# AER-RC/RRTMG_LW

Measured on AMD Instinct MI355X. Metric: columns/sec, 72-layer profiles, higher is better.
Workload: dtype f64 (transmittance / tfn codes and their LDS table f32); 1 GPU; 1000000 synthetic 72-layer columns, config 'cloudy' (icld=2: rtrnmr max-random overlap, idrv=0), sharded 1x1000000; ncol_total=1000000, nlay=72, columns_per_gpu=1000000, parallelism=columns/1, gather=none, kdata=stand-in (real k-data absent from the reference mount), sweeps=production

## Files before the change

### rrtmg_lw_amd/csrc/driver.hip

```cpp
#include <hip/hip_runtime.h>
#include <cstdlib>
#include <sched.h>

#include <algorithm>
#include <array>
#include <atomic>
#include <cstdint>
#include <cstdarg>
#include <mutex>
#include <string>
#include <chrono>
#include <condition_variable>
#include <functional>
#include <map>
#include <thread>
#include <type_traits>
#include <vector>

#include "../../include/rrtmg_lw_hip.h"
#include "kernels.hip"
#include "mtjump.hpp"
#include "hostrows.hpp"
#include "owned.hpp"

// ... 2 lines not shown
using namespace rrlw;

constexpr int BLOCK = 256;
const int HOST_BATCH = []() { const char *e = getenv("RRTMG_LW_HOST_BATCH"); const int v = e ? atoi(e) : 0; return v >= 64 ? v : 16384; }();

constexpr int HOST_SETS = 4;

struct DevMemTraits {
    using handle = void *;
    static int acquire(void **p, size_t bytes) { return (int)hipMalloc(p, bytes); }
    static int release(void *p) { const hipError_t s = hipDeviceSynchronize(), f = hipFree(p); return (int)(s != hipSuccess ? s : f); }
};
struct PinnedTraits {
    using handle = void *;
    static int acquire(void **p, size_t bytes) { return (int)hipHostMalloc(p, bytes, hipHostMallocDefault); }
    static int release(void *p) { return (int)hipHostFree(p); }
};
struct StreamTraits { using handle = hipStream_t; static int release(hipStream_t s) { return (int)hipStreamDestroy(s); } };
struct EventTraits { using handle = hipEvent_t; static int release(hipEvent_t e) { return (int)hipEventDestroy(e); } };
struct GraphTraits { using handle = hipGraph_t; static int release(hipGraph_t g) { return (int)hipGraphDestroy(g); } };
struct GraphExecTraits { using handle = hipGraphExec_t; static int release(hipGraphExec_t g) { return (int)hipGraphExecDestroy(g); } };
using DevBuf = owned::GrowBuf<DevMemTraits>;
using PinnedBuf = owned::GrowBuf<PinnedTraits>;
using Stream = owned::Owned<StreamTraits>;
using Event = owned::Owned<EventTraits>;
using Graph = owned::Owned<GraphTraits>;
using GraphExec = owned::Owned<GraphExecTraits>;

constexpr int KISS_SLOTS = 2 * RRTMG_LW_HIP_MAX_SAMPLES;
struct KissSlot { unsigned long long stride = 0; long long seed = -1; unsigned long long used = 0; };
struct KissTable { std::vector<KissSlot> slot; unsigned long long clock = 0; DevBuf dev; PinnedBuf host; };

constexpr int DEFAULT_BATCH = 262144;
struct State {
    bool init = false;
    int device = -1;
    HostTables H;
    DevTables D;
    DevBuf d_ktab, d_stat;
    Workspace W{};
    DevBuf ws_buf;
    struct WsShape {
        int nlay = 0, ncolb = 0;
        bool cloud = false, mc = false, gdp = false, efcl = false, ovl = false;
        bool two_scr = false;
        int groups = 0;
        size_t slabcols = 0;
    } ws;
    DevBuf opt_buf;
    int opt_nlay = 0, opt_ncolb = 0;
    double *opt_percol = nullptr;
    int *opt_laytrop = nullptr, *opt_wide = nullptr;
    DevBuf d_err;
    struct PrepSet { double *percol; int *laytrop, *ncbands; double *odcld, *efcl; int *cflag; int *btop, *order, *hgrp, *hblk, *bbot, *hbot; double2 *ovl; int *perm, *wsort; double *tlayc, *tlevc, *cldfc; int *wide; } prep[2] = {};
    struct ScrSet { unsigned *scr[NSCR]; unsigned *fw; } scrset[2] = {};
    Stream aux;
    struct SweepSet { Stream main, q[3]; Event go, done[3]; } swset[2];
    Stream lay_u, lay_m;
    int cu_layer = 0;
    int cu_total = 0;
    bool sweep_fanout = true;
    Event ev_last;
    Event ev_fork, ev_join;
    bool ev_last_valid = false;
    Event ev_in, ev_ready[2], ev_layer[2], ev_done[2];
    DevBuf mask;
    DevBuf d_rnd;
    bool batch_set = false;
    int batch = DEFAULT_BATCH;
    bool split_sweep = false;
    bool sweep_attrs = false;
    bool n1 = false;
    DevBuf stage_buf;
    DevBuf form_buf, form_gen;
    Stream stream;
    Stream cp_in, cp_out;
    PinnedBuf h_tot;
    struct HostSet { PinnedBuf in, out, fill, widen, narrow; } hset[HOST_SETS];
    Event ev_h2d[HOST_SETS], ev_cmp[HOST_SETS], ev_d2h[HOST_SETS];
    KissTable kiss;
    std::string err;
    bool profile = false;
    struct GraphEnt { std::vector<unsigned char> key; GraphExec exec; int seen = 0; bool failed = false; unsigned long long used = 0; };
    std::vector<GraphEnt> graphs;
    unsigned long long graph_clock = 0;
    Stream cap;
    long long graph_replays = 0, graph_captures = 0;
    unsigned long long init_gen = 0;
    struct ProfRec { const char *name; Event a, b; };
    std::vector<ProfRec> prof;
    std::vector<Event> evpool;
};
constexpr int MAXDEV = 16;
owned::NoDestroy<std::array<State, MAXDEV>> g_states_store;
std::array<State, MAXDEV> &g_states = g_states_store.get();
int g_ndev = 1;
thread_local State *g_cur = &g_states[0];
#define G (*g_cur)
std::mutex g_mu;

struct CallDesc {
    int ncol, nlay;
    int *icld;
    int idrv, inflg, iceflg, liqflg;
    int permuteseed = 0; int *irng = nullptr;
    bool spectral = false;
    size_t esz = 8;
// ... 345 lines not shown

void graphs_clear();
int g_split_max = []() { const char *e = getenv("RRTMG_LW_SPLIT_MAX"); return e ? std::max(0, atoi(e)) : 768; }();
int ensure_workspace(int nlay, int ncolb, bool cloud, bool mc = false, int idrv = 1, int mode = -1)
{
    SweepGroups fgw;
    int groups = NGROUP_MAX;
    if (mode >= 0 && make_groups(mode, idrv, 1, NBND, fgw)) groups = fgw.n;
    const bool gdp = idrv == 1, efcl = cloud && (mode < 0 || mode == 1 || mode == 3), ovl = cloud && (mode < 0 || mode == 2);
    const size_t split_cols = ncolb <= g_split_max ? (size_t)NBND * align_up((size_t)ncolb, 64) : 0;
    const State::WsShape &have = G.ws;
    if (G.ws_buf && have.nlay == nlay && have.ncolb >= ncolb && (have.cloud || !cloud) && (have.mc || !mc) && (have.two_scr || !G.split_sweep) &&
        have.groups >= groups && have.slabcols >= split_cols && (have.gdp || !gdp) && (have.efcl || !efcl) && (have.ovl || !ovl)) return 0;
    if (G.ws_buf) { HIP_TRY(hipDeviceSynchronize()); graphs_clear(); if (int rc = drop(G.ws_buf, "workspace")) return rc; }
    const bool same = have.nlay == nlay;
    ncolb = std::max(ncolb, same ? have.ncolb : 0);
    cloud = cloud || have.cloud || mc;
    mc = mc || have.mc;
    const int ng = std::max(groups, have.groups);
    const bool want_gdp = gdp || have.gdp, want_efcl = efcl || have.efcl, want_ovl = ovl || have.ovl;
    const size_t n = (size_t)ncolb, L = (size_t)nlay;
    const size_t slabcols = std::max((size_t)ng * n, (size_t)NBND * align_up(std::min(n, (size_t)std::max(g_split_max, 0)), 64));
    struct Item { void **p; size_t bytes; };
    Workspace &W = G.W;
    W = Workspace{};
    std::vector<Item> items = {
        {(void **)&W.gdn1, slabcols * (L + 1) * sizeof(double)},
        {(void **)&W.gup1, slabcols * (L + 1) * sizeof(double)},
        {(void **)&W.gup, slabcols * (L + 1) * sizeof(Part2)},
        {(void **)&W.gdn, slabcols * (L + 1) * sizeof(Part2)},
    };
    if (want_gdp) items.push_back({(void **)&W.gdp, slabcols * (L + 1) * sizeof(Part2)});
    const bool two_scr = G.split_sweep;
    G.scrset[1] = State::ScrSet{};
    for (int k = 0; k < (two_scr ? 2 : 1); k++) {
        State::ScrSet &ss = G.scrset[k];
        ss = State::ScrSet{};
        items.push_back({(void **)&ss.scr[S_CODE], (size_t)NQUAD * L * n * CODE_BYTES});
        items.push_back({(void **)&ss.fw, (size_t)NFW * L * n * sizeof(unsigned)});
        if (cloud) items.push_back({(void **)&ss.scr[S_CODET], (size_t)NQUAD * L * n * CODE_BYTES});
    }
    for (auto &ps : G.prep) {
        ps = State::PrepSet{};
        items.push_back({(void **)&ps.percol, (size_t)NPERCOL * n * 8});
        items.push_back({(void **)&ps.laytrop, n * 4});
        items.push_back({(void **)&ps.ncbands, n * 4});
        items.push_back({(void **)&ps.cflag, (L + 2) * n * 4});
        const size_t nblk = (n + 63) / 64, nslot = (size_t)sort_slots((int)nblk);
        items.push_back({(void **)&ps.btop, nblk * 4});
        items.push_back({(void **)&ps.hblk, nblk * 4});
        items.push_back({(void **)&ps.order, nslot * 4});
        items.push_back({(void **)&ps.hgrp, (nslot / SORT_GROUP) * 4});
        items.push_back({(void **)&ps.bbot, nblk * 4});
        items.push_back({(void **)&ps.hbot, (nslot / SORT_GROUP) * 4});
        items.push_back({(void **)&ps.perm, align_up(n, COLSORT_WIN) * 4});
        items.push_back({(void **)&ps.wsort, (align_up(n, COLSORT_WIN) / COLSORT_WIN) * 4});
        items.push_back({(void **)&ps.wide, (2 + ((n + LAYER_BLOCK - 1) / LAYER_BLOCK) * L) * 4});
        if (cloud) {
            items.push_back({(void **)&ps.tlayc, L * n * 8});
            items.push_back({(void **)&ps.tlevc, (L + 1) * n * 8});
            items.push_back({(void **)&ps.cldfc, L * n * 8});
        }
    }
    if (cloud) items.push_back({(void **)&W.hand, (size_t)5 * NQUAD * 4 * n * 8});
    if (cloud) {
        for (auto &ps : G.prep) {
            items.push_back({(void **)&ps.odcld, 16 * L * n * 8});
            if (want_efcl) items.push_back({(void **)&ps.efcl, 16 * L * n * 8});
            if (want_ovl) items.push_back({(void **)&ps.ovl, (size_t)2 * (L + 1) * 3 * n * sizeof(double2)});
        }
    }
    if (mc) {
        items.push_back({(void **)&W.odg, (size_t)NQUAD * 4 * L * n * 8});
        items.push_back({(void **)&W.cfef, (size_t)NQUAD * 8 * L * n * 4});
    }
    size_t total = 0;
    for (auto &it : items) total += align_up(it.bytes, 256);
    if (int rc = grow(G.ws_buf, total, total, "workspace")) return rc;
    size_t off = 0;
    for (auto &it : items) { *it.p = G.ws_buf.as<char>() + off; off += align_up(it.bytes, 256); }
    for (auto &ps : G.prep) HIP_TRY(hipMemset(ps.wide, 0, 8));
    W.ncolb = ncolb;
    W.pcb = ncolb;
    W.nlay = nlay;
    W.err = G.d_err.as<int>();
    for (int a = 0; a < NSCR; a++) W.scr[a] = G.scrset[0].scr[a];
    W.fw = G.scrset[0].fw;
    {
        const State::PrepSet &ps = G.prep[0];
        W.percol = ps.percol; W.laytrop = ps.laytrop; W.ncbands = ps.ncbands; W.cflag = ps.cflag;
        W.odcld = ps.odcld; W.efcl = ps.efcl; W.ovl = ps.ovl;
        W.btop = ps.btop; W.order = ps.order; W.hgrp = ps.hgrp; W.hblk = ps.hblk; W.bbot = ps.bbot; W.hbot = ps.hbot;
    }
    G.ws = State::WsShape{nlay, ncolb, cloud, mc, want_gdp, want_efcl, want_ovl, two_scr, ng, slabcols};
    return 0;
}

int ensure_mask(int nlay, size_t ncol)
{
    const size_t bytes = (size_t)KJ_NWORD * nlay * ncol * sizeof(unsigned);
    return grow(G.mask, bytes, bytes, "sub-column masks");
}

bool g_colsort = []() { const char *e = getenv("RRTMG_LW_COLSORT"); return !e || atoi(e) != 0; }();
bool use_colsort(bool gcm, int mode, int nb);
constexpr int COLSORT_NEVER = 1 << 24;
int g_colsort_min = []() { const char *e = getenv("RRTMG_LW_COLSORT_MIN"); return e ? std::max(0, std::min(atoi(e), COLSORT_NEVER)) : 24; }();
constexpr int COLSORT_CLEAR_MAX = 1000;
constexpr int COLSORT_CLEAR_DEFAULT = 18;
int g_colsort_clear = []() { const char *e = getenv("RRTMG_LW_COLSORT_CLEAR"); return e ? std::max(0, std::min(atoi(e), COLSORT_CLEAR_MAX)) : COLSORT_CLEAR_DEFAULT; }();
bool g_clear_groups = []() { const char *e = getenv("RRTMG_LW_CLEAR_GROUPS"); return !e || atoi(e) != 0; }();

Workspace ws_for(int k, bool sorted)
{
    Workspace w = G.W;
    const State::PrepSet &ps = G.prep[k];
    w.perm = sorted ? ps.perm : nullptr;
    w.wsort = sorted ? ps.wsort : nullptr;
    w.tlayc = ps.tlayc; w.tlevc = ps.tlevc; w.cldfc = ps.cldfc;
    w.wide = ps.wide;
    w.percol = ps.percol; w.laytrop = ps.laytrop; w.ncbands = ps.ncbands; w.cflag = ps.cflag;
    w.odcld = ps.odcld; w.efcl = ps.efcl; w.ovl = ps.ovl;
    w.btop = ps.btop; w.order = ps.order; w.hgrp = ps.hgrp; w.hblk = ps.hblk; w.bbot = ps.bbot; w.hbot = ps.hbot;
    const State::ScrSet &ss = G.scrset[G.ws.two_scr ? k : 0];
    for (int a = 0; a < NSCR; a++) w.scr[a] = ss.scr[a];
    w.fw = ss.fw;
    return w;
}

int make_stream(Stream &st, int lo, int hi)
{
    if (hi <= lo) { HIP_TRY(hipStreamCreateWithFlags(st.slot(), hipStreamNonBlocking)); return 0; }
    uint32_t mask[32] = {};
    const int nw = (G.cu_total + 31) / 32;
    for (int b = lo; b < hi && b < 1024; b++) mask[b >> 5] |= 1u << (b & 31);
    HIP_TRY(hipExtStreamCreateWithCUMask(st.slot(), (uint32_t)nw, mask));
    return 0;
}
int ensure_sweep_set(int k)
{
    if (G.swset[k].q[0]) return 0;
    const int lo = k == 1 ? G.cu_layer : 0, hi = k == 1 ? G.cu_total : 0;
    State::SweepSet SS;
    if (int rc = make_stream(SS.main, lo, hi)) return rc;
    for (int j = 0; j < 3; j++) {
        if (int rc = make_stream(SS.q[j], lo, hi)) return rc;
        if (int rc = make_event(SS.done[j])) return rc;
    }
    if (int rc = make_event(SS.go)) return rc;
    G.swset[k] = std::move(SS);
    return 0;
}

int g_one_sweep_max = []() { const char *e = getenv("RRTMG_LW_ONE_SWEEP_MAX"); return e ? atoi(e) : 4096; }();
bool one_sweep(int nb, int mode) { return mode != 0 && nb <= g_one_sweep_max; }
bool g_wide_window = []() { const char *e = getenv("RRTMG_LW_WIDE_WINDOW"); return !e || atoi(e) != 0; }();
bool g_prep_fork = []() { const char *e = getenv("RRTMG_LW_PREP_FORK"); return !e || atoi(e) != 0; }();
bool g_layer_split = []() { const char *e = getenv("RRTMG_LW_LAYER_SPLIT"); return !e || atoi(e) != 0; }();
bool use_colsort(bool gcm, int mode, int nb) { return g_colsort && gcm && (mode == 1 || mode == 2 || mode == 3) && !one_sweep(nb, mode); }

template <bool GCM>
int run_prep(hipStream_t s, const Workspace &Wk, const Batch &b, const GcmIn &g, const ColIn &c, hipStream_t side = nullptr)
{
    const dim3 cgrid1((b.nb + 63) / 64), cblock1(64);
    if (Wk.perm) {
        const dim3 wgrid((b.nb + COLSORT_WIN - 1) / COLSORT_WIN);
        LAUNCH("k_colsort", (k_colsort<GCM>), wgrid, dim3(COLSORT_WIN, COLSORT_TY), s, Wk, g, c, b.nb, b.col0, b.nct, g_colsort_min, (int)((long long)Wk.nlay * g_colsort_clear / 100));
    }
    const bool scan = b.mode == 1 || b.mode == 2, fork = scan && side && side != s;
    if (fork) {
        HIP_TRY(hipEventRecord(G.ev_fork.get(), s));
        HIP_TRY(hipStreamWaitEvent(side, G.ev_fork.get(), 0));
    }
    LAUNCH("k_colprep", (k_colprep<GCM>), cgrid1, cblock1, fork ? side : s, G.D, Wk, g, c, b.nb, b.col0, b.nct, b.idrv, b.istart, scan ? 0 : 1);
    if (fork) HIP_TRY(hipEventRecord(G.ev_join.get(), side));
    if (scan) {
// ... 3809 lines not shown
```

### rrtmg_lw_amd/csrc/kernels.hip

```cpp
#include <hip/hip_runtime.h>
#include "kissjump.hpp"

#ifdef RRLW_TUNE
#define RRLW_BF_TUNE 1u
#else
#define RRLW_BF_TUNE 0u
#endif
#ifdef RRLW_G256
#define RRLW_BF_G256 8u
#else
#define RRLW_BF_G256 0u
#endif
#if defined(RRLW_LAYER_BLOCK) || defined(RRLW_STAGE_DOUBLES) || defined(RRLW_LAYER_WAVES) || defined(RRLW_LOAD_CHUNK) || defined(RRLW_MINOR_WIN) || \
    defined(RRLW_COLSORT_WIN) || defined(RRLW_SWEEPC_P0) || defined(RRLW_SWEEPC_P2D) || defined(RRLW_SWEEPC_WAVES_CAP) || defined(RRLW_SWEEPC_CODES) || \
    defined(RRLW_SWEEPZ_WAVES_G1) || defined(RRLW_SWEEPZ_WAVES_IDRV) || defined(RRLW_LAYER_STAMPS) || \
    defined(RRLW_DBG_DUMP)
#define RRLW_BF_GEOMETRY 16u
#else
#define RRLW_BF_GEOMETRY 0u
#endif

#include <algorithm>
#include <type_traits>
#include <utility>

#include "tables.hpp"

namespace rrlw {

constexpr unsigned BUILD_FLAGS = RRLW_BF_TUNE | RRLW_BF_G256 | RRLW_BF_GEOMETRY;

struct DevTables {
    const double *ktab;
    const double *stat;
    BandLayout band[NBND];
    StaticLayout sl;
    double absice0[2], abscld1, absliq0;
    double delwave[NBND];
    double refrat[NBND][6];
    double heatfac, fluxfac, oneminus, bpade;
};

enum Field {
    F_FAC00, F_FAC01, F_FAC10, F_FAC11,
    F_COLH2O, F_COLCO2, F_COLO3, F_COLN2O, F_COLCO, F_COLCH4, F_COLO2, F_COLBRD,
    F_COLDRY, F_SELFFAC, F_SELFFRAC, F_FORFAC, F_FORFRAC, F_MINORFRAC, F_SCALEMINOR, F_SCALEMINORN2,
    F_PAVEL, F_WX1, F_WX2, F_WX3, F_WX4,
    NFIELD
};
enum PerCol { PC_PLANKBND = 0, PC_DPLANKBND = 16, PC_SECDIFF = 32, NPERCOL = 48 };
enum Scr { S_CODE, S_CODET, NSCR };
struct alignas(16) Part2 { double a, b; };

typedef float scr_t;
constexpr int CODE_WORDS = 4;
constexpr int CODE_BYTES = 4 * CODE_WORDS;

struct Workspace {
    int ncolb;
    int nlay;
    double *percol;
    int *laytrop;
    int *ncbands;
    double *odcld;
    double *efcl;
    int *cflag;
    double2 *ovl;
    int *btop;
    int *order;
    int *hgrp;
    int *hblk;
    int *bbot;
    int *hbot;
    double *hand;
    unsigned *scr[NSCR];
    unsigned *fw;
    double *gdn1, *gup1;
    Part2 *gup, *gdp, *gdn;
    int pcb;
    int *err;
    double *odg;
    float *cfef;
    unsigned *mask;
    size_t mask_stride;
    size_t mask_col0;
    int *wide;
    int *perm;
    int *wsort;
    double *tlayc, *tlevc, *cldfc;
};
#ifndef RRLW_COLSORT_WIN
#define RRLW_COLSORT_WIN 256
#endif
constexpr int COLSORT_WIN = RRLW_COLSORT_WIN;
__device__ __forceinline__ bool pmoved(const Workspace &W, int slot) { return W.perm && W.wsort[__builtin_amdgcn_readfirstlane(slot) / COLSORT_WIN] != 0; }
__device__ __forceinline__ int pcol(const Workspace &W, int slot)
{
    if (!W.perm) return slot;
    const int moved = W.wsort[__builtin_amdgcn_readfirstlane(slot) / COLSORT_WIN];
    return moved ? W.perm[slot] : slot;
}
__device__ __forceinline__ double col_load(const double *row, unsigned off8)
{
    typedef unsigned int u32x2c __attribute__((ext_vector_type(2)));
    const u32x2c v = __builtin_amdgcn_raw_buffer_load_b64(__builtin_amdgcn_make_buffer_rsrc(const_cast<double *>(row), 0, 0x7ffffff0, 0x00020000), (int)off8, 0, 0);
    double r;
    __builtin_memcpy(&r, &v, 8);
    return r;
}

struct GcmIn {
    const double *play, *plev, *tlay, *tlev, *tsfc, *h2ovmr, *o3vmr, *co2vmr, *ch4vmr, *n2ovmr, *o2vmr;
    const double *cfc11vmr, *cfc12vmr, *cfc22vmr, *ccl4vmr, *emis;
    const double *cldfr, *taucld, *cicewp, *cliqwp, *reice, *reliq, *tauaer;
    const double *tauctot = nullptr;
};
struct ColIn {
    const double *pavel, *tavel, *pz, *tz, *tbound, *semiss, *coldry, *wkl, *wbrodl, *wx, *pwvcm;
    const double *cldfrac, *tauc, *ciwp, *clwp, *rei, *rel, *taua;
};
struct McIn {
    const double *cldfmcl, *taucmcl, *ciwpmcl, *clwpmcl;
    const double *reicmcl, *relqmcl;
};
struct FluxOut {
    double *uflx, *dflx, *hr, *uflxc, *dflxc, *hrc, *duflx_dt, *duflxc_dt;
    double *fnet, *fnetc;
    double *uflxs, *dflxs, *uflxcs, *dflxcs;
    double *uflx_var, *dflx_var, *hr_var;
};
struct OptOut {
    double *taug = nullptr, *fracs = nullptr, *planklay = nullptr, *planklev = nullptr, *plankbnd = nullptr, *dplankbnd = nullptr;
};

enum ErrCode { E_NONE = 0, E_ICE_SMALL = 1, E_ICE_BOUNDS = 2, E_ICE_GEN_BOUNDS = 3, E_LIQ_BOUNDS = 4, E_BAD_FLAG = 5,
               E_MC_INFLAG1 = 6, E_KISS_PMID = 7 };

__device__ __forceinline__ int clampi(int v, int lo, int hi) { return v < lo ? lo : (v > hi ? hi : v); }

__device__ __forceinline__ double fdiv(double a, double b)
{
    double r = __builtin_amdgcn_rcp(b);
    r = fma(fma(-b, r, 1.0), r, r);
    const double q = a * r;
    return fma(fma(-b, q, a), r, q);
}

constexpr int COLSORT_TY = 4;
template <bool GCM>
__global__ __launch_bounds__(COLSORT_WIN * COLSORT_TY) void k_colsort(Workspace W, GcmIn g, ColIn c, int ncol, int col0, int nct, int min_gain, int clear_bonus)
{
    constexpr int NB = COLSORT_WIN / 64;
    __shared__ int s_key[COLSORT_WIN], s_perm[COLSORT_WIN], s_top[COLSORT_TY][COLSORT_WIN];
    __shared__ int s_nat[NB], s_srt[NB];
    const int t = threadIdx.x, ty = threadIdx.y, w0 = blockIdx.x * COLSORT_WIN, col = w0 + t;
    const int nlay = W.nlay;
    int top = -1;
    if (col < ncol) {
        const double *cf = (GCM ? g.cldfr : c.cldfrac) + (size_t)col0 + col;
        const int per = (nlay + COLSORT_TY - 1) / COLSORT_TY, l0 = ty * per + 1, l1 = min(nlay, l0 + per - 1);
        top = 0;
#pragma unroll 8
        for (int lay = l0; lay <= l1; lay++) { if (cf[(size_t)nct * (lay - 1)] >= 1.e-6) top = lay; }
    }
    s_top[ty][t] = top;
    __syncthreads();
    int rank = 0;
    if (ty == 0) {
#pragma unroll
        for (int k = 1; k < COLSORT_TY; k++) top = max(top, s_top[k][t]);
        s_key[t] = (nlay - top) * COLSORT_WIN + t;
        int mx = max(top, 0);
#pragma unroll
        for (int o = 32; o >= 1; o >>= 1) mx = max(mx, __shfl_xor(mx, o, 64));
        if ((t & 63) == 0) s_nat[t >> 6] = mx;
    }
    __syncthreads();
    if (ty == 0) {
        const int key = s_key[t];
#pragma unroll 8
        for (int i = 0; i < COLSORT_WIN; i++) rank += s_key[i] < key ? 1 : 0;
        if ((rank & 63) == 0) s_srt[rank >> 6] = max(top, 0);
    }
    __syncthreads();
    int gain = 0;
#pragma unroll
    for (int b = 0; b < NB; b++) gain += s_nat[b] - s_srt[b] + ((s_srt[b] == 0 && s_nat[b] != 0) ? clear_bonus : 0);
    const bool keep = gain * 4 < min_gain * NB;
    if (ty == 0) {
        if (keep) rank = t;
        if (t == 0) W.wsort[blockIdx.x] = keep ? 0 : 1;
        W.perm[w0 + rank] = col;
// ... 23 lines not shown
    const size_t gc = (size_t)col0 + pcol(W, col);
    const int nlay = W.nlay;
    const double *S = T.stat;
    const double *totplnk = S + T.sl.totplnk, *totplnkd = S + T.sl.totplnkderiv;
    const double *totplk16 = S + T.sl.totplk16, *totplk16d = S + T.sl.totplk16deriv;
    const double amd = 28.9660, amw = 18.0160, avogad = 6.02214199e+23, grav = 9.8066;

    const double tbound = GCM ? g.tsfc[gc] : c.tbound[gc];
    const double pz0 = GCM ? g.plev[gc] : c.pz[gc];
    const int indbound = clampi((int)(tbound - 159.), 1, 180);
    const double tbndfrac = tbound - 159. - (double)indbound;
#pragma unroll
    for (int b = 0; b < NBND; b++) {
        const double semiss = GCM ? g.emis[gc + (size_t)nct * b] : c.semiss[gc + (size_t)nct * b];
        const double *tp = (b == 15 && istart == 16) ? totplk16 : totplnk + 181 * b;
        const double *td = (b == 15 && istart == 16) ? totplk16d : totplnkd + 181 * b;
        const double pb = semiss * (tp[indbound - 1] + tbndfrac * (tp[indbound] - tp[indbound - 1]));
        double dpb = 0.0;
        if (idrv == 1) dpb = semiss * (td[indbound - 1] + tbndfrac * (td[indbound] - td[indbound - 1]));
        W.percol[(size_t)(PC_PLANKBND + b) * W.ncolb + col] = pb;
        W.percol[(size_t)(PC_DPLANKBND + b) * W.ncolb + col] = dpb;
    }
    double amttl = 0.0, wvttl = 0.0, pzlo = pz0;
    int laytrop = 0;
#pragma unroll 8
    for (int lay = 1; lay <= nlay; lay++) {
        const size_t gi = gc + (size_t)nct * (lay - 1);
        const double pavel = GCM ? g.play[gi] : c.pavel[gi];
        if (!(log(pavel) <= 4.56)) laytrop++;
        if (GCM) {
            const double w1v = g.h2ovmr[gi];
            const double pzl = g.plev[gc + (size_t)nct * lay];
            const double amm = (1. - w1v) * amd + w1v * amw;
            const double coldry = (pzlo - pzl) * 1.e3 * avogad / (1.e2 * grav * amm * (1. + w1v));
            pzlo = pzl;
            const double w1 = coldry * w1v;
            amttl = amttl + coldry + w1;
            wvttl = wvttl + w1;
        }
    }
    W.laytrop[col] = laytrop;
    double pwvcm;
    if (GCM) {
        const double wvsh = (amw * wvttl) / (amd * amttl);
        pwvcm = wvsh * (1.e3 * pz0) / (1.e2 * grav);
    } else {
        pwvcm = c.pwvcm[gc];
    }
    const double a0[16] = {1.66, 1.55, 1.58, 1.66, 1.54, 1.454, 1.89, 1.33, 1.668, 1.66, 1.66, 1.66, 1.66, 1.66, 1.66, 1.66};
    const double a1[16] = {0.00, 0.25, 0.22, 0.00, 0.13, 0.446, -0.10, 0.40, -0.006, 0.00, 0.00, 0.00, 0.00, 0.00, 0.00, 0.00};
    const double a2[16] = {0.00, -12.0, -11.7, 0.00, -0.72, -0.243, 0.19, -0.062, 0.414, 0.00, 0.00, 0.00, 0.00, 0.00, 0.00, 0.00};
#pragma unroll
    for (int b = 0; b < NBND; b++) {
        double sd = 1.66;
        if (!(b == 0 || b == 3 || b >= 9)) {
            sd = a0[b] + a1[b] * exp(a2[b] * pwvcm);
            if (sd > 1.80) sd = 1.80;
            if (sd < 1.50) sd = 1.50;
        }
        W.percol[(size_t)(PC_SECDIFF + b) * W.ncolb + col] = sd;
    }
    if (init_cloud) {
        W.ncbands[col] = 1;
        W.cflag[col] = 0;
        if ((col & 63) == 0) { W.btop[col >> 6] = 0; W.bbot[col >> 6] = nlay + 1; }
    }
}

__device__ __forceinline__ int icb_map(int ib, int ind)
{
    if (ind == 0) return 1;
    if (ind == 2) return ib;
    return ib <= 2 ? ib : (ib <= 5 ? 3 : (ib <= 8 ? 4 : 5));
}

__device__ __forceinline__ bool cloud_layer_enters(double cf, double cwp, double tauctot)
{
    const double cldmin = 1.e-20;
    return cf >= cldmin && (cwp >= cldmin || tauctot >= cldmin);
}
template <bool GCM>
__device__ __forceinline__ double cloud_tauctot(const GcmIn &g, const ColIn &c, size_t gc, size_t gi, int nct, int lay)
{
    if constexpr (GCM) { if (g.tauctot) return g.tauctot[gi]; }
    double tauctot = 0.0;
    for (int ib = 0; ib < NBND; ib++)
        tauctot = tauctot + (GCM ? g.taucld[ib + (size_t)NBND * gi] : c.tauc[gc + (size_t)nct * (ib + (size_t)NBND * (lay - 1))]);
    return tauctot;
}

struct OvlFac { double clr1, cld1, cmb1, cmb2, clr2, cld2; bool rat1, rat2; };
__device__ __forceinline__ OvlFac mr_step(double cl, double cn, double cp, bool first, bool last, bool brat1, bool brat2)
{
    const double rat1 = brat1 ? 1. : 0., rat2 = brat2 ? 1. : 0.;
    const bool act = !last, up = cn >= cl;
    const double fmx = fmax(cl, cp), fmn = fmin(cl, cp);
    const bool u_f = act && up && first && cl < 1.;
    const bool u_gt = act && up && !first && cn > fmx;
    const bool u_lt = act && up && !first && cn < fmx;
    const bool u_eq = act && up && !first && !(cn > fmx) && !(cn < fmx);
    const bool d_f = act && !up && first;
    const bool d_le = act && !up && !first && cn <= fmn;
    const bool d_gt = act && !up && !first && !(cn <= fmn);
    double num = 0.0, den = 1.0;
    num = u_f ? cn - cl : num;     den = u_f ? 1. - cl : den;
    num = u_gt ? cn - fmx : num;   den = u_gt ? 1. - fmx : den;
    num = u_lt ? cn - cl : num;    den = u_lt ? cp - cl : den;
    num = d_f ? cl - cn : num;     den = d_f ? cl : den;
    num = d_le ? fmn - cn : num;   den = d_le ? fmn : den;
    num = d_gt ? cl - cn : num;    den = d_gt ? cl - fmn : den;
    const double q = fdiv(num, den);
    const double clr1 = (u_gt || u_eq) ? rat2 : (u_lt ? q : 0.0);
    const double clr2 = (u_f || u_gt) ? q : 0.0;
    const double cld1 = d_le ? rat1 : (d_gt ? q : 0.0);
    const double cld2 = (d_f || d_le) ? q : 0.0;
    const bool r1 = (act && up) ? (clr1 > 0. || clr2 > 0.) : (act ? false : brat1);
    const bool r2 = (act && !up) ? (cld1 > 0. || cld2 > 0.) : (act ? false : brat2);
    double cmb1 = 0.0, cmb2 = 0.0;
    if (!first) {
        const double cx = last ? 0.0 : cn;
        cmb1 = fmax(0., fmin(cx - cl, cp - cl));
        cmb2 = fmax(0., fmin(cl - cx, cl - cp));
    }
    return OvlFac{clr1, cld1, cmb1, cmb2, clr2, cld2, r1, r2};
}

template <bool GCM>
__global__ __launch_bounds__(256) void k_cloudscan(Workspace W, GcmIn g, ColIn c, int ncol, int col0, int nct, int inflag, int iceflag, int liqflag, int mode)
{
    const int col = blockIdx.x * blockDim.x + threadIdx.x;
    const int nlay = W.nlay;
    int top = 0, bot = nlay + 1;
    if (col < ncol) {
    const size_t gc = (size_t)col0 + pcol(W, col);
    const double *cldfr = GCM ? g.cldfr : c.cldfrac;
    const double *ciwp_ = GCM ? g.cicewp : c.ciwp, *clwp_ = GCM ? g.cliqwp : c.clwp;
    int ncbands = 1, anycloud = 0;
    const size_t ncb = W.ncolb;
    bool prevcld = false, rat1 = false, rat2 = false;
    double cfprev = 0.0;
#pragma unroll 4
    for (int lay = 1; lay <= nlay; lay++) {
        const size_t gi = gc + (size_t)nct * (lay - 1);
        const double cf = cldfr[gi], ciwp = ciwp_[gi], clwp = clwp_[gi];
        const double cwp = ciwp + clwp;
        bool enters = cf >= 1.e-20 && cwp >= 1.e-20;
        if (cf >= 1.e-20 && !enters) enters = cloud_layer_enters(cf, cwp, cloud_tauctot<GCM>(g, c, gc, gi, nct, lay));
        if (enters) {
            if (inflag == 0 || inflag == 1) ncbands = 16;
            else if (inflag == 2) {
                if (ciwp != 0.0) { if (iceflag == 1) ncbands = 5; else if (iceflag == 2 || iceflag == 3) ncbands = 16; }
                if (clwp != 0.0 && liqflag == 1) ncbands = 16;
            }
        }
        const int cloudy = cf >= 1.e-6;
        if (cloudy && !anycloud) bot = lay;
        anycloud |= cloudy;
        if (cloudy) top = lay;
        int first = 0;
        if (mode == 2) {
            if (cloudy) {
                first = !prevcld;
                const OvlFac mf = mr_step(cf, lay < nlay ? cldfr[gi + nct] : 0.0, cfprev, first, lay == nlay, rat1, rat2);
                rat1 = mf.rat1; rat2 = mf.rat2;
                prevcld = true;
                cfprev = cf;
                double2 *o = W.ovl + ((size_t)((nlay + 1) + lay) * 3) * ncb + col;
                o[0] = make_double2(mf.clr1, mf.cld1); o[ncb] = make_double2(mf.cmb1, mf.cmb2); o[2 * ncb] = make_double2(mf.clr2, mf.cld2);
            } else prevcld = false;
        }
        W.cflag[(size_t)lay * ncb + col] = cloudy | (first << 2) | (ncbands << 8);
    }
    if (mode == 2 && anycloud) {
        prevcld = false; rat1 = false; rat2 = false; cfprev = 0.0;
        for (int lay = top; lay >= 1; lay--) {
            const size_t gi = gc + (size_t)nct * (lay - 1);
            const double cf = cldfr[gi];
            if (cf >= 1.e-6) {
                const bool first = !prevcld;
                const OvlFac mf = mr_step(cf, lay > 1 ? cldfr[gi - nct] : 0.0, cfprev, first, lay == 1, rat1, rat2);
                rat1 = mf.rat1; rat2 = mf.rat2;
                prevcld = true;
                cfprev = cf;
                double2 *o = W.ovl + ((size_t)lay * 3) * ncb + col;
                o[0] = make_double2(mf.clr1, mf.cld1); o[ncb] = make_double2(mf.cmb1, mf.cmb2); o[2 * ncb] = make_double2(mf.clr2, mf.cld2);
                if (first) W.cflag[(size_t)lay * ncb + col] |= 2;
            } else prevcld = false;
        }
    }
    W.ncbands[col] = ncbands;
    W.cflag[col] = anycloud ? 8 : 0;
    W.cflag[(size_t)(nlay + 1) * W.ncolb + col] = 0;
    }
#pragma unroll
    for (int o = 32; o >= 1; o >>= 1) { top = max(top, __shfl_xor(top, o, 64)); bot = min(bot, __shfl_xor(bot, o, 64)); }
    if (threadIdx.x == 0 && col < ncol) { W.btop[col >> 6] = top; W.bbot[col >> 6] = bot; }
}

template <bool GCM>
__global__ __launch_bounds__(256) void k_cloudlay(DevTables T, Workspace W, GcmIn g, ColIn c, int ncol, int col0, int nct, int mode,
                                                  int inflag, int iceflag, int liqflag)
{
    const int col = blockIdx.x * blockDim.x + threadIdx.x;
    if (col >= ncol) return;
    const int lay = blockIdx.y + 1;
    const size_t gc = (size_t)col0 + pcol(W, col);
    const int nlay = W.nlay;
    const size_t ncb = W.ncolb;
    const size_t gi = gc + (size_t)nct * (lay - 1);
    const double *S = T.stat;
    const double *absice1 = S + T.sl.absice1, *absice2 = S + T.sl.absice2, *absice3 = S + T.sl.absice3, *absliq1 = S + T.sl.absliq1;
    const double cf = (GCM ? g.cldfr : c.cldfrac)[gi];
    const double ciwp = (GCM ? g.cicewp : c.ciwp)[gi], clwp = (GCM ? g.cliqwp : c.clwp)[gi];
    const int flagword = W.cflag[(size_t)lay * ncb + col];
    const int cloudy = flagword & 1, nb_at = flagword >> 8;
    const int ncbands = W.ncbands[col];
    const double cwp = ciwp + clwp;
    bool enters = cf >= 1.e-20 && cwp >= 1.e-20;
    if (cf >= 1.e-20 && !enters) enters = cloud_layer_enters(cf, cwp, cloud_tauctot<GCM>(g, c, gc, gi, nct, lay));
    int err = 0, icemode = -1, liqmode = -1, iceind = 0, liqind = 0, index_i = 1, index_l = 1;
    double radice = 0.0, ice_single = 0.0, fint_i = 0.0, liq_single = 0.0, fint_l = 0.0;
    if (enters && inflag == 2) {
        radice = (GCM ? g.reice : c.rei)[gi];
        if (ciwp == 0.0) { icemode = 0; ice_single = 0.0; iceind = 0; }
        else if (iceflag == 0) {
            if (radice < 10.0) err = E_ICE_SMALL;
            icemode = 0; ice_single = T.absice0[0] + T.absice0[1] / radice; iceind = 0;
        } else if (iceflag == 1) {
            if (radice < 13.0 || radice > 130.) err = E_ICE_BOUNDS;
            icemode = 1; iceind = 1;
        } else if (iceflag == 2) {
            if (radice < 5.0 || radice > 131.0) err = E_ICE_BOUNDS;
            const double factor = (radice - 2.) / 3.;
            index_i = (int)factor; if (index_i == 43) index_i = 42;
            fint_i = factor - (double)index_i;
            icemode = 2; iceind = 2;
        } else if (iceflag == 3) {
            if (radice < 5.0 || radice > 140.0) err = E_ICE_GEN_BOUNDS;
            const double factor = (radice - 2.) / 3.;
            index_i = (int)factor; if (index_i == 46) index_i = 45;
            fint_i = factor - (double)index_i;
            icemode = 3; iceind = 2;
        } else err = E_BAD_FLAG;
        if (clwp == 0.0) { liqmode = 0; liq_single = 0.0; liqind = 0; if (iceind == 1) iceind = 2; }
        else if (liqflag == 0) { liqmode = 0; liq_single = T.absliq0; liqind = 0; if (iceind == 1) iceind = 2; }
        else if (liqflag == 1) {
            const double radliq = (GCM ? g.reliq : c.rel)[gi];
            if ((radliq < 2.5 || radliq > 60.) && !err) err = E_LIQ_BOUNDS;
            index_l = (int)(radliq - 1.5);
            if (index_l == 0) index_l = 1;
            if (index_l == 58) index_l = 57;
            fint_l = radliq - 1.5 - (double)index_l;
            liqmode = 1; liqind = 2;
        } else err = E_BAD_FLAG;
        if (err) index_i = clampi(index_i, 1, 42), index_l = clampi(index_l, 1, 57);
    }
    if (err) atomicCAS(W.err, 0, err);
    if (!cloudy) return;
// ... 965 lines not shown
                                            const double2 *lds, int jp0, int im0, bool ok, bool lower, int lay, int col, bool incol, const OptOut &o)
{
    unsigned delta[NROLE];
    const bool use_lds = __builtin_amdgcn_ballot_w64(!ok) == 0ull;
    const unsigned off8 = incol ? (unsigned)col * 8u : 0x80000000u;
    if (lower) {
        constexpr int N = region_nrows(BT<B>::lo, true);
        Rows<N> rw;
        rows_prep<B, true, N>(T, C, rw);
        if (use_lds) {
            band_delta<B, true, WN, BASE_LO>(T, jp0, im0, delta);
            rows_to_lds<B, true, N>(rw, delta);
            optics_cells<B, true, N, true>(T, W, a, C, kt, lds, rw, lay, off8, o);
        } else {
            optics_cells<B, true, N, false>(T, W, a, C, kt, lds, rw, lay, off8, o);
        }
    } else {
        constexpr int N = region_nrows(BT<B>::up, false);
        Rows<N> rw;
        rows_prep<B, false, N>(T, C, rw);
        if constexpr (B == 16) {
            const unsigned tab = (unsigned)T.band[B - 1].absb, ng = (unsigned)BT<B>::ng;
            rw.off[0] = tab; rw.off[1] = tab + ng; rw.off[2] = tab; rw.off[3] = tab + ng;
            optics_cells<B, false, N, false>(T, W, a, C, kt, lds, rw, lay, off8, o);
        } else if (use_lds) {
            band_delta<B, false, WN, BASE_UP>(T, jp0, im0, delta);
            rows_to_lds<B, false, N>(rw, delta);
            optics_cells<B, false, N, true>(T, W, a, C, kt, lds, rw, lay, off8, o);
        } else {
            optics_cells<B, false, N, false>(T, W, a, C, kt, lds, rw, lay, off8, o);
        }
    }
}

#ifndef RRLW_LAYER_WAVES
#define RRLW_LAYER_WAVES 3
#endif

struct LayerWg { double2 *lds; int jp0, im0, tid, nth, pc; bool lower, ok; };

template <int B, int CLOUD, class WN, int BASE_LO, int BASE_UP>
__device__ __forceinline__ void layer_band(const DevTables &T, const Workspace &W, const LayerArgs &a, const LayerCoef &C,
                                           __amdgpu_buffer_rsrc_t kt, const LayerWg &wg, bool lower, int lay, int col, bool incol, int cloudy,
                                           const unsigned (&mw)[MASK_WORDS])
{
    STAMP(4);
    unsigned delta[NROLE];
#pragma unroll
    for (int r = 0; r < NROLE; r++) delta[r] = 0u;
    const bool use_lds = __builtin_amdgcn_ballot_w64(!wg.ok) == 0ull;
    const size_t ncb = W.ncolb, gcx = (size_t)a.col0 + wg.pc;
    double odcld = 0.0;
    if constexpr (CLOUD == 1 || CLOUD == 3 || CLOUD == CL_SHARE) { if (cloudy) odcld = W.odcld[((size_t)(B - 1) * W.nlay + (lay - 1)) * ncb + col]; }
    const double secdiff = W.percol[(size_t)(PC_SECDIFF + B - 1) * ncb + col];
    const double taua = col_load(a.tauaer + (size_t)a.col0 + (size_t)a.nct * ((lay - 1) + (size_t)W.nlay * (B - 1)), (unsigned)wg.pc * 8u);
    unsigned gbits = 0u;
    if constexpr (CLOUD == 3 || CLOUD == CL_SHARE) {
        (void)mw;
        constexpr int g0 = band_g0(B), ng = BT<B>::ng, w0 = g0 >> 5, w1 = (g0 + ng - 1) >> 5;
        if (cloudy) {
            const unsigned *mrow = W.mask + (size_t)(lay - 1) * W.mask_stride + W.mask_col0 + gcx;
            const unsigned long long lo = mrow[(size_t)w0 * W.nlay * W.mask_stride];
            const unsigned long long hi = w1 != w0 ? mrow[(size_t)w1 * W.nlay * W.mask_stride] : 0u;
            gbits = (unsigned)(((lo | (hi << 32)) >> (g0 & 31)) & ((1ull << ng) - 1ull));
        }
    }
    if (lower) {
        constexpr int N = region_nrows(BT<B>::lo, true);
        Rows<N> rw;
        rows_prep<B, true, N>(T, C, rw);
        if (use_lds) {
            band_delta<B, true, WN, BASE_LO>(T, wg.jp0, wg.im0, delta);
            rows_to_lds<B, true, N>(rw, delta);
            STAMP(2);
            band_cells<B, CLOUD, true, N, true>(T, W, kt, wg.lds, rw, lay, col, incol, secdiff, taua, cloudy, odcld, gbits);
        } else {
            band_cells<B, CLOUD, true, N, false>(T, W, kt, wg.lds, rw, lay, col, incol, secdiff, taua, cloudy, odcld, gbits);
        }
    } else {
        constexpr int N = region_nrows(BT<B>::up, false);
        Rows<N> rw;
        rows_prep<B, false, N>(T, C, rw);
        if (use_lds) {
            band_delta<B, false, WN, BASE_UP>(T, wg.jp0, wg.im0, delta);
            rows_to_lds<B, false, N>(rw, delta);
            STAMP(2);
            band_cells<B, CLOUD, false, N, true>(T, W, kt, wg.lds, rw, lay, col, incol, secdiff, taua, cloudy, odcld, gbits);
        } else {
            band_cells<B, CLOUD, false, N, false>(T, W, kt, wg.lds, rw, lay, col, incol, secdiff, taua, cloudy, odcld, gbits);
        }
    }
}

#ifdef RRLW_G256
using LayerPasses = std::tuple<BandList<1, 2, 11, 15, 6>, BandList<8, 10, 14, 16>, BandList<12>, BandList<13>, BandList<4, 9>, BandList<7>, BandList<3>, BandList<5>>;
#else
using LayerPasses = std::tuple<BandList<1, 2, 11, 15, 6, 8, 10, 14, 16, 12, 13>, BandList<4, 9>, BandList<7, 3>, BandList<5>>;
#endif
#ifdef RRLW_G256
using LayerPassesWide = LayerPasses;
#else
using LayerPassesWide = std::tuple<BandList<1, 2, 11, 15, 6, 8, 10, 14, 16, 13>, BandList<12, 4>, BandList<9>, BandList<7>, BandList<3>, BandList<5>>;
#endif

template <class PL, class WN, int CLOUD, int... I>
__device__ __forceinline__ void pass_run(std::integer_sequence<int, I...>, const DevTables &T, const Workspace &W, const LayerArgs &a,
                                         const LayerCoef &C, __amdgpu_buffer_rsrc_t kt, const LayerWg &wg, bool lower, int lay, int col, bool incol,
// ... 1026 lines not shown
    const size_t i = (size_t)blockIdx.x * blockDim.x + threadIdx.x;
    if (i >= (size_t)a.ncol) return;
    const int nlay = a.nlay;
    if (a.nbat) {
        int ncbands = a.imca ? NBND : 1;
        if (!a.imca) {
#pragma unroll 4
            for (int k = 0; k < nlay; k++) {
                const size_t at = co_lay(a, i, k);
                const double cf = co_get<R>(a.cldfr, at), ciwp = co_get<R>(a.cicewp, at), clwp = co_get<R>(a.cliqwp, at);
                const double cwp = ciwp + clwp;
                bool enters = cf >= 1.e-20 && cwp >= 1.e-20;
                if (cf >= 1.e-20 && !enters) enters = co_tauctot<R>(a, i, k) >= 1.e-20;
                if (enters) {
                    if (a.inflag == 0 || a.inflag == 1) ncbands = 16;
                    else if (a.inflag == 2) {
                        if (ciwp != 0.0) { if (a.iceflag == 1) ncbands = 5; else if (a.iceflag == 2 || a.iceflag == 3) ncbands = 16; }
                        if (clwp != 0.0 && a.liqflag == 1) ncbands = 16;
                    }
                }
                a.nbat[(size_t)k * a.ncol + i] = (unsigned char)ncbands;
            }
        }
        a.nbat[(size_t)nlay * a.ncol + i] = (unsigned char)ncbands;
        if (a.ncbands) a.ncbands[i] = ncbands;
    }
    if (!a.secdiff) return;
    const double amd = 28.9660, amw = 18.0160, avogad = 6.02214199e+23, grav = 9.8066;
    const size_t nlev = (size_t)nlay + 1;
    const auto lev_at = [&](int k) {
        const size_t kk = (size_t)(a.top_first ? nlay - k : k);
        return a.layer_fastest ? i * nlev + kk : i + a.ld * kk;
    };
    const double pz0 = co_get<R>(a.plev, lev_at(0));
    double amttl = 0.0, wvttl = 0.0, pzlo = pz0;
#pragma unroll 8
    for (int k = 0; k < nlay; k++) {
        const double w1v = co_get<R>(a.h2ovmr, co_lay(a, i, k));
        const double pzl = co_get<R>(a.plev, lev_at(k + 1));
        const double amm = (1. - w1v) * amd + w1v * amw;
        const double coldry = (pzlo - pzl) * 1.e3 * avogad / (1.e2 * grav * amm * (1. + w1v));
        pzlo = pzl;
        const double w1 = coldry * w1v;
        amttl = amttl + coldry + w1;
        wvttl = wvttl + w1;
    }
    const double wvsh = (amw * wvttl) / (amd * amttl);
    const double pwvcm = wvsh * (1.e3 * pz0) / (1.e2 * grav);
    const double a0[16] = {1.66, 1.55, 1.58, 1.66, 1.54, 1.454, 1.89, 1.33, 1.668, 1.66, 1.66, 1.66, 1.66, 1.66, 1.66, 1.66};
    const double a1[16] = {0.00, 0.25, 0.22, 0.00, 0.13, 0.446, -0.10, 0.40, -0.006, 0.00, 0.00, 0.00, 0.00, 0.00, 0.00, 0.00};
    const double a2[16] = {0.00, -12.0, -11.7, 0.00, -0.72, -0.243, 0.19, -0.062, 0.414, 0.00, 0.00, 0.00, 0.00, 0.00, 0.00, 0.00};
#pragma unroll
    for (int b = 0; b < NBND; b++) {
        double sd = 1.66;
        if (!(b == 0 || b == 3 || b >= 9)) {
            sd = a0[b] + a1[b] * exp(a2[b] * pwvcm);
            if (sd > 1.80) sd = 1.80;
            if (sd < 1.50) sd = 1.50;
        }
        static_cast<R *>(a.secdiff)[a.layer_fastest ? i * NBND + b : i + a.ld * b] = (R)sd;
    }
}

template <class R>
__global__ __launch_bounds__(256) void k_cloudoptics(DevTables T, CloudOpticsArgs a)
{
#pragma clang fp contract(off)
    const size_t i = (size_t)blockIdx.x * blockDim.x + threadIdx.x;
    if (i >= (size_t)a.ncol) return;
    const int k = blockIdx.y, nlay = a.nlay;
    const double *S = T.stat;
    const double *absice1 = S + T.sl.absice1, *absice2 = S + T.sl.absice2, *absice3 = S + T.sl.absice3, *absliq1 = S + T.sl.absliq1;
    const double cldmin = 1.e-20;
    const size_t at = co_lay(a, i, k);
    const double cf = co_get<R>(a.cldfr, at), ciwp = co_get<R>(a.cicewp, at), clwp = co_get<R>(a.cliqwp, at);
    const double cwp = ciwp + clwp;
    const int inflag = a.inflag, iceflag = a.iceflag, liqflag = a.liqflag;
    const size_t kk = (size_t)(a.top_first ? nlay - 1 - k : k);
    const auto put = [&](int B, double v) {
        if (a.taucloud) static_cast<R *>(a.taucloud)[a.layer_fastest ? (i * (size_t)nlay + kk) * NBND + (B - 1) : i + a.ld * (kk + (size_t)nlay * (B - 1))] = (R)v;
    };
    int err = 0;
    bool formed = false;
    if (!a.imca) {
        bool enters = cf >= cldmin && cwp >= cldmin;
        if (cf >= cldmin && !enters) enters = co_tauctot<R>(a, i, k) >= cldmin;
        if (enters) {
            formed = true;
            const int nb_at = a.nbat[(size_t)k * a.ncol + i], ncbands = a.nbat[(size_t)nlay * a.ncol + i];
            int icemode = -1, liqmode = -1, iceind = 0, liqind = 0, index_i = 1, index_l = 1;
            double radice = 0.0, ice_single = 0.0, fint_i = 0.0, liq_single = 0.0, fint_l = 0.0;
            if (inflag == 2) {
                radice = co_get<R>(a.reice, at);
                if (ciwp == 0.0) { icemode = 0; ice_single = 0.0; iceind = 0; }
                else if (iceflag == 0) {
                    if (radice < 10.0) err = E_ICE_SMALL;
                    icemode = 0; ice_single = T.absice0[0] + T.absice0[1] / radice; iceind = 0;
                } else if (iceflag == 1) {
                    if (radice < 13.0 || radice > 130.) err = E_ICE_BOUNDS;
                    icemode = 1; iceind = 1;
                } else if (iceflag == 2) {
                    if (radice < 5.0 || radice > 131.0) err = E_ICE_BOUNDS;
                    const double factor = (radice - 2.) / 3.;
                    index_i = (int)factor; if (index_i == 43) index_i = 42;
                    fint_i = factor - (double)index_i;
                    index_i = clampi(index_i, 1, 42);
                    icemode = 2; iceind = 2;
                } else if (iceflag == 3) {
// ... 311 lines not shown
    const int hgrp = (PHASE == 0 && !a.cfree) ? 0 : __builtin_amdgcn_readfirstlane(W.hgrp[(blockIdx.x * blockDim.z) / SORT_GROUP]);
    if (a.cfree && (PHASE == 0) != (hgrp == 0)) return;
    const int tx = threadIdx.x, ty = __builtin_amdgcn_readfirstlane(threadIdx.y), sub = __builtin_amdgcn_readfirstlane(threadIdx.z);
    const int bi = ty / NT, part = ty % NT;
    const int ny = blockDim.y, nb = ny / NT, nsb = blockDim.z, ncw = 64 * nsb;
    const float2 *s_lut = reinterpret_cast<const float2 *>(smem);
    double (*s_pl)[184] = reinterpret_cast<double (*)[184]>(smem + SWEEP_LUT_BYTES + bi * SWEEPC_BAND_BYTES);
    double (*s_fr)[16] = reinterpret_cast<double (*)[16]>(smem + SWEEP_LUT_BYTES + bi * SWEEPC_BAND_BYTES + SWEEP_PL_BYTES);
    double *red = reinterpret_cast<double *>(smem + SWEEP_LUT_BYTES + nb * SWEEPC_BAND_BYTES);
    const int slot = blockIdx.x * nsb + sub;
    const int cblock = (PHASE == 0 && !a.cfree) ? slot : __builtin_amdgcn_readfirstlane(W.order[slot]);
    const int col = cblock * 64 + tx;
    const int bsel = a.split ? (int)blockIdx.y : 0;
    const unsigned long long bands = a.bands >> (4 * bsel);
    const int B = (int)((bands >> (4 * bi)) & 15ull) + 1;
    const bool incol = col < a.ncol;
    const int colc = incol ? col : a.ncol - 1;
    const int quad = __builtin_amdgcn_readfirstlane(band_qstart(B) + part * G);
    const int g0 = NG * part;
    const int pc = pcol(W, colc);
    const size_t gc = (size_t)a.col0 + pc;
    const int nlay = W.nlay, nct = a.nct;
    const size_t ncb = W.ncolb;
    const bool alt16 = (B == 16 && a.istart == 16);
    const bool lo_bin = (LO_BINARY >> (B - 1)) & 1u, up_bin = (UP_BINARY >> (B - 1)) & 1u;
    const bool any_bin = lo_bin || up_bin;
    const int base_up = ((UP_ZERO >> (B - 1)) & 1u) ? 14 : (((UP_FROM_A >> (B - 1)) & 1u) ? 0 : 9);
    sweep_stage_lut(T, smem, (sub * ny + ty) * 64 + tx, 64 * ny * nsb);
    sweep_stage_band(T, s_pl, s_fr, B, alt16, lo_bin, up_bin, (sub * NT + part) * 64 + tx, NT * ncw);
    __syncthreads();
    const int lo = PHASE == 0 ? 1 : hgrp + 1;
    const size_t qstride = (size_t)nlay * ncb;
    const unsigned *__restrict__ sC = W.scr[S_CODE] + (size_t)quad * qstride * CODE_WORDS;
    const unsigned *__restrict__ sFw = W.fw + (size_t)fw_slot(B) * nlay * ncb;
    const bool moved = pmoved(W, colc);
    const double *__restrict__ tlay = moved ? W.tlayc : a.tlay + a.col0;
    const double *__restrict__ tlev = moved ? W.tlevc : a.tlev + a.col0;
    const size_t tstride = moved ? ncb : (size_t)nct;
    const unsigned offc = (unsigned)colc * (unsigned)CODE_BYTES, off8p = (unsigned)colc * 8u, off4 = (unsigned)colc * 4u;
    const size_t pcb = (size_t)W.pcb;
    const size_t gslab = (size_t)(a.group + bsel) * (nlay + 1) * pcb;
    double *__restrict__ gdn1 = W.gdn1 + gslab;
    double *__restrict__ gup1 = W.gup1 + gslab;
    Part2 *__restrict__ gup = W.gup + gslab;
    Part2 *__restrict__ gdp = W.gdp + gslab;
    const unsigned so8 = (unsigned)col * 8u, so16 = (unsigned)col * 16u;
    const int laytrop = W.laytrop[colc];
    const double *tp0 = s_pl[0], *tp1 = s_pl[1];
    double2 *hand = reinterpret_cast<double2 *>(W.hand) + ((size_t)quad * ncb + colc) * 2;
    const size_t hstream = (size_t)NQUAD * ncb * 2;

    constexpr bool SOFF = PHASE != 1;
    const unsigned ncb32 = (unsigned)ncb, tstr32 = (unsigned)tstride;
    auto fill_t = [&](auto bin_tag, int lev, int zoff, SweepcLev<G> &q) {
        const int l = min(max(lev, 1), nlay);
        if constexpr (SOFF) {
            const unsigned r = (unsigned)(l - 1);
            q.tl = bload_f64(row_ptr(tlay, r, tstr32), off8p);
            q.tz = bload_f64(row_ptr(tlev, r + (unsigned)zoff, tstr32), off8p);
            if constexpr (decltype(bin_tag)::value) q.w = bload_u32(sFw, off4, r * ncb32 * 4u);
        } else {
            q.tl = bload_f64(tlay + tstride * (l - 1), off8p);
            q.tz = bload_f64(tlev + tstride * (l - 1 + zoff), off8p);
            if constexpr (decltype(bin_tag)::value) q.w = bload_u32(sFw + (size_t)(l - 1) * ncb, off4);
        }
    };
    auto ld_c = [&](int lev, int k) -> pk4 {
        const int l = min(max(lev, 1), nlay);
        if constexpr (SOFF) return bload_pk4_nt(sC + (size_t)k * qstride * CODE_WORDS, offc, (unsigned)(l - 1) * ncb32 * (unsigned)CODE_BYTES);
        else return bload_pk4_nt(sC + ((size_t)k * qstride + (size_t)(l - 1) * ncb) * CODE_WORDS, offc);
    };
    auto frac_row = [&](int lev, unsigned fwv, double &fpl) -> const double * {
        const bool lower = lev <= laytrop;
        if (any_bin) {
            const unsigned w = (lower ? lo_bin : up_bin) ? fwv : 0x10000000u;
            const int r0 = clampi((lower ? 0 : base_up) + (int)(w >> 28) - 1, 0, 14);
            fpl = (double)(w & 0x0fffffffu) * (1.0 / 268435456.0);
            return &s_fr[r0][g0];
        }
        fpl = 0.0;
        return &s_fr[lower ? 0 : base_up][g0];
    };

    const unsigned rlane = (unsigned)(sub * 64 + tx);
    const unsigned vstride = (unsigned)(ny * NC * ncw), rband = (unsigned)(ty * NC * ncw);
    unsigned bufoff = 0u;
    auto red_put = [&](int c, int val, double v) { red[bufoff + val * vstride + rband + (unsigned)(c * ncw) + rlane] = v; };
    auto round_end = [&](auto dn_tag, int lev0, int nvalid) {
#pragma clang fp contract(off)
        constexpr bool DN = decltype(dn_tag)::value;
        constexpr int NV = DN ? 1 : NVAL;
        __syncthreads();
        for (int c = ty; c < nvalid; c += ny) {
            const int lvl = DN ? lev0 - c - 1 : lev0 + c;
            double sv[NV];
#pragma unroll
            for (int val = 0; val < NV; val++) {
                const double *r = red + (bufoff + val * vstride + (unsigned)(c * ncw) + rlane);
                const bool deriv = IDRV && !DN && val >= (TWO ? 2 : 1);
                double sum = 0.0;
                for (int q = 0; q < nb; q++) {
                    double pq = r[(unsigned)(q * NT * NC * ncw)];
                    if constexpr (NT == 2) pq = pq + r[(unsigned)((q * NT + 1) * NC * ncw)];
                    const int bq = (int)((bands >> (4 * q)) & 15ull);
                    double v = (pq * 0.5) * T.delwave[bq];
                    if (deriv) v = v * T.fluxfac;
                    sum = q == 0 ? v : sum + v;
                    if constexpr (SPEC) {
                        if (incol && !deriv) {
                            const size_t o = spec_at(gc, lvl, bq + 1, nlay, nct);
                            const double f = v * T.fluxfac;
                            if (DN) { a.dflxs[o] = f; if (a.dflxcs) a.dflxcs[o] = f; }
                            else if (val == 0) { a.uflxs[o] = f; if (!TWO && a.uflxcs) a.uflxcs[o] = f; }
                            else if (a.uflxcs) a.uflxcs[o] = f;
                        }
                    }
                }
// ... 1642 lines not shown
```

Baseline: 18.13 million columns/s.

## Skip clear-layer cloud optics blocks, constant secdiff literals, cap upper fw loads

```diff
diff --git a/rrtmg_lw_amd/csrc/driver.hip b/rrtmg_lw_amd/csrc/driver.hip
--- a/rrtmg_lw_amd/csrc/driver.hip
+++ b/rrtmg_lw_amd/csrc/driver.hip
@@ -78,7 +78,7 @@
     double *opt_percol = nullptr;
     int *opt_laytrop = nullptr, *opt_wide = nullptr;
     DevBuf d_err;
-    struct PrepSet { double *percol; int *laytrop, *ncbands; double *odcld, *efcl; int *cflag; int *btop, *order, *hgrp, *hblk, *bbot, *hbot; double2 *ovl; int *perm, *wsort; double *tlayc, *tlevc, *cldfc; int *wide; } prep[2] = {};
+    struct PrepSet { double *percol; int *laytrop, *ncbands; double *odcld, *efcl; int *cflag; int *btop, *order, *hgrp, *hblk, *bbot, *hbot, *betop; double2 *ovl; int *perm, *wsort; double *tlayc, *tlevc, *cldfc; int *wide; } prep[2] = {};
     struct ScrSet { unsigned *scr[NSCR]; unsigned *fw; } scrset[2] = {};
     Stream aux;
     struct SweepSet { Stream main, q[3]; Event go, done[3]; } swset[2];
@@ -530,6 +530,7 @@
         items.push_back({(void **)&ps.order, nslot * 4});
         items.push_back({(void **)&ps.hgrp, (nslot / SORT_GROUP) * 4});
         items.push_back({(void **)&ps.bbot, nblk * 4});
+        items.push_back({(void **)&ps.betop, nblk * 4});
         items.push_back({(void **)&ps.hbot, (nslot / SORT_GROUP) * 4});
         items.push_back({(void **)&ps.perm, align_up(n, COLSORT_WIN) * 4});
         items.push_back({(void **)&ps.wsort, (align_up(n, COLSORT_WIN) / COLSORT_WIN) * 4});
@@ -568,7 +569,7 @@
         const State::PrepSet &ps = G.prep[0];
         W.percol = ps.percol; W.laytrop = ps.laytrop; W.ncbands = ps.ncbands; W.cflag = ps.cflag;
         W.odcld = ps.odcld; W.efcl = ps.efcl; W.ovl = ps.ovl;
-        W.btop = ps.btop; W.order = ps.order; W.hgrp = ps.hgrp; W.hblk = ps.hblk; W.bbot = ps.bbot; W.hbot = ps.hbot;
+        W.btop = ps.btop; W.order = ps.order; W.hgrp = ps.hgrp; W.hblk = ps.hblk; W.bbot = ps.bbot; W.hbot = ps.hbot; W.betop = ps.betop;
     }
     G.ws = State::WsShape{nlay, ncolb, cloud, mc, want_gdp, want_efcl, want_ovl, two_scr, ng, slabcols};
     return 0;
@@ -599,7 +600,7 @@
     w.wide = ps.wide;
     w.percol = ps.percol; w.laytrop = ps.laytrop; w.ncbands = ps.ncbands; w.cflag = ps.cflag;
     w.odcld = ps.odcld; w.efcl = ps.efcl; w.ovl = ps.ovl;
-    w.btop = ps.btop; w.order = ps.order; w.hgrp = ps.hgrp; w.hblk = ps.hblk; w.bbot = ps.bbot; w.hbot = ps.hbot;
+    w.btop = ps.btop; w.order = ps.order; w.hgrp = ps.hgrp; w.hblk = ps.hblk; w.bbot = ps.bbot; w.hbot = ps.hbot; w.betop = ps.betop;
     const State::ScrSet &ss = G.scrset[G.ws.two_scr ? k : 0];
     for (int a = 0; a < NSCR; a++) w.scr[a] = ss.scr[a];
     w.fw = ss.fw;
diff --git a/rrtmg_lw_amd/csrc/kernels.hip b/rrtmg_lw_amd/csrc/kernels.hip
--- a/rrtmg_lw_amd/csrc/kernels.hip
+++ b/rrtmg_lw_amd/csrc/kernels.hip
@@ -71,6 +71,7 @@
     int *hgrp;
     int *hblk;
     int *bbot;
+    int *betop;
     int *hbot;
     double *hand;
     unsigned *scr[NSCR];
@@ -138,6 +139,14 @@
 
 __device__ __forceinline__ int clampi(int v, int lo, int hi) { return v < lo ? lo : (v > hi ? hi : v); }
 
+constexpr double SECDIFF_CONST = 1.66;
+__host__ __device__ constexpr bool secdiff_is_const(int b) { return b == 0 || b == 3 || b >= 9; }
+#ifdef RRLW_G256
+constexpr bool SECDIFF_LITERAL = false;
+#else
+constexpr bool SECDIFF_LITERAL = true;
+#endif
+
 __device__ __forceinline__ double fdiv(double a, double b)
 {
     double r = __builtin_amdgcn_rcp(b);
@@ -267,8 +276,8 @@
     const double a2[16] = {0.00, -12.0, -11.7, 0.00, -0.72, -0.243, 0.19, -0.062, 0.414, 0.00, 0.00, 0.00, 0.00, 0.00, 0.00, 0.00};
 #pragma unroll
     for (int b = 0; b < NBND; b++) {
-        double sd = 1.66;
-        if (!(b == 0 || b == 3 || b >= 9)) {
+        double sd = SECDIFF_CONST;
+        if (!secdiff_is_const(b)) {
             sd = a0[b] + a1[b] * exp(a2[b] * pwvcm);
             if (sd > 1.80) sd = 1.80;
             if (sd < 1.50) sd = 1.50;
@@ -345,7 +354,7 @@
 {
     const int col = blockIdx.x * blockDim.x + threadIdx.x;
     const int nlay = W.nlay;
-    int top = 0, bot = nlay + 1;
+    int top = 0, bot = nlay + 1, etop = 0;
     if (col < ncol) {
     const size_t gc = (size_t)col0 + pcol(W, col);
     const double *cldfr = GCM ? g.cldfr : c.cldfrac;
@@ -362,6 +371,7 @@
         bool enters = cf >= 1.e-20 && cwp >= 1.e-20;
         if (cf >= 1.e-20 && !enters) enters = cloud_layer_enters(cf, cwp, cloud_tauctot<GCM>(g, c, gc, gi, nct, lay));
         if (enters) {
+            etop = lay;
             if (inflag == 0 || inflag == 1) ncbands = 16;
             else if (inflag == 2) {
                 if (ciwp != 0.0) { if (iceflag == 1) ncbands = 5; else if (iceflag == 2 || iceflag == 3) ncbands = 16; }
@@ -408,8 +418,8 @@
     W.cflag[(size_t)(nlay + 1) * W.ncolb + col] = 0;
     }
 #pragma unroll
-    for (int o = 32; o >= 1; o >>= 1) { top = max(top, __shfl_xor(top, o, 64)); bot = min(bot, __shfl_xor(bot, o, 64)); }
-    if (threadIdx.x == 0 && col < ncol) { W.btop[col >> 6] = top; W.bbot[col >> 6] = bot; }
+    for (int o = 32; o >= 1; o >>= 1) { top = max(top, __shfl_xor(top, o, 64)); bot = min(bot, __shfl_xor(bot, o, 64)); etop = max(etop, __shfl_xor(etop, o, 64)); }
+    if (threadIdx.x == 0 && col < ncol) { W.btop[col >> 6] = top; W.bbot[col >> 6] = bot; W.betop[col >> 6] = etop; }
 }
 
 template <bool GCM>
@@ -417,8 +427,14 @@
                                                   int inflag, int iceflag, int liqflag)
 {
     const int col = blockIdx.x * blockDim.x + threadIdx.x;
+    const int lay = blockIdx.y + 1;
+    {
+        const int b0 = blockIdx.x * (blockDim.x >> 6), nbw = min((int)(blockDim.x >> 6), ((ncol + 63) >> 6) - b0);
+        int lim = 0;
+        for (int k = 0; k < nbw; k++) lim = max(lim, max(W.btop[b0 + k], W.betop[b0 + k]));
+        if (lay > lim) return;
+    }
     if (col >= ncol) return;
-    const int lay = blockIdx.y + 1;
     const size_t gc = (size_t)col0 + pcol(W, col);
     const int nlay = W.nlay;
     const size_t ncb = W.ncolb;
@@ -1490,7 +1506,8 @@
     const size_t ncb = W.ncolb, gcx = (size_t)a.col0 + wg.pc;
     double odcld = 0.0;
     if constexpr (CLOUD == 1 || CLOUD == 3 || CLOUD == CL_SHARE) { if (cloudy) odcld = W.odcld[((size_t)(B - 1) * W.nlay + (lay - 1)) * ncb + col]; }
-    const double secdiff = W.percol[(size_t)(PC_SECDIFF + B - 1) * ncb + col];
+    double secdiff = SECDIFF_CONST;
+    if constexpr (!(SECDIFF_LITERAL && secdiff_is_const(B - 1))) secdiff = W.percol[(size_t)(PC_SECDIFF + B - 1) * ncb + col];
     const double taua = col_load(a.tauaer + (size_t)a.col0 + (size_t)a.nct * ((lay - 1) + (size_t)W.nlay * (B - 1)), (unsigned)wg.pc * 8u);
     unsigned gbits = 0u;
     if constexpr (CLOUD == 3 || CLOUD == CL_SHARE) {
@@ -2623,8 +2640,8 @@
     const double a2[16] = {0.00, -12.0, -11.7, 0.00, -0.72, -0.243, 0.19, -0.062, 0.414, 0.00, 0.00, 0.00, 0.00, 0.00, 0.00, 0.00};
 #pragma unroll
     for (int b = 0; b < NBND; b++) {
-        double sd = 1.66;
-        if (!(b == 0 || b == 3 || b >= 9)) {
+        double sd = SECDIFF_CONST;
+        if (!secdiff_is_const(b)) {
             sd = a0[b] + a1[b] * exp(a2[b] * pwvcm);
             if (sd > 1.80) sd = 1.80;
             if (sd < 1.50) sd = 1.50;
@@ -3042,17 +3059,24 @@
 
     constexpr bool SOFF = PHASE != 1;
     const unsigned ncb32 = (unsigned)ncb, tstr32 = (unsigned)tstride;
+    int lcap = nlay;
+    if (any_bin && !up_bin) {
+        int m = laytrop;
+#pragma unroll
+        for (int o = 32; o >= 1; o >>= 1) m = max(m, __shfl_xor(m, o, 64));
+        lcap = min(max(__builtin_amdgcn_readfirstlane(m), 1), nlay);
+    }
     auto fill_t = [&](auto bin_tag, int lev, int zoff, SweepcLev<G> &q) {
-        const int l = min(max(lev, 1), nlay);
+        const int l = min(max(lev, 1), nlay), lw = min(l, lcap);
         if constexpr (SOFF) {
             const unsigned r = (unsigned)(l - 1);
             q.tl = bload_f64(row_ptr(tlay, r, tstr32), off8p);
             q.tz = bload_f64(row_ptr(tlev, r + (unsigned)zoff, tstr32), off8p);
-            if constexpr (decltype(bin_tag)::value) q.w = bload_u32(sFw, off4, r * ncb32 * 4u);
+            if constexpr (decltype(bin_tag)::value) q.w = bload_u32(sFw, off4, (unsigned)(lw - 1) * ncb32 * 4u);
         } else {
             q.tl = bload_f64(tlay + tstride * (l - 1), off8p);
             q.tz = bload_f64(tlev + tstride * (l - 1 + zoff), off8p);
-            if constexpr (decltype(bin_tag)::value) q.w = bload_u32(sFw + (size_t)(l - 1) * ncb, off4);
+            if constexpr (decltype(bin_tag)::value) q.w = bload_u32(sFw + (size_t)(lw - 1) * ncb, off4);
         }
     };
     auto ld_c = [&](int lev, int k) -> pk4 {
```

After: 17.93 million columns/s. -1.1%, worse.
